# usnistgov/alignn

Measured on AMD Instinct MI355X. Metric: graphs/sec (train fwd+bwd), batch=64 JARVIS-DFT crystals, 4+4 ALIGNN layers, higher is better.
Workload: dtype f32 (projections: split-product MFMA - 3 fp16-slice or 6 bf16-slice products, fp32 accumulate, fp32-grade error)

## Files before the change

alignn_amd/csrc/gemm_dw.hip:

```cpp
#include <type_traits>
#include <utility>

#include "common.h"
#include "../../include/alignn_hip.h"

#ifndef DW_ABL
#define DW_ABL 0
#endif
#ifndef DW_TRACE
#define DW_TRACE 0
#endif
#ifndef DW_NS
#define DW_NS 4
#endif
#ifndef DW_IL
#define DW_IL 0
#endif
#ifndef DW_PP
#define DW_PP 0
#endif
#if DW_TRACE
__device__ unsigned long long dw_trace_buf[256 * 16];
#endif

#ifndef DW_GRID_DEFAULT
#define DW_GRID_DEFAULT 224
#endif

namespace {

typedef float f32x16 __attribute__((ext_vector_type(16)));
typedef _Float16 f16x8 __attribute__((ext_vector_type(8)));
typedef short s16x4 __attribute__((__vector_size__(4 * sizeof(short))));
typedef short s16x8 __attribute__((__vector_size__(8 * sizeof(short))));

constexpr int H = 256;
constexpr int R = 64;
constexpr int NW = 8, NTH = NW * 64;
constexpr int NS = DW_NS;
constexpr int SLOT = 16384;
constexpr int GBUF = 0;
constexpr int RING = GBUF + R * 1024;
constexpr int PATCH = RING + NS * SLOT;
constexpr int PLD = 68, PATCH_W = 8 * PLD * 4;
constexpr int NSTAT = PATCH + NW * PATCH_W;
constexpr int LDS_BYTES = NSTAT + 4 * H * 4;
static_assert(LDS_BYTES <= 160 * 1024, "one workgroup per CU");

template <int NE>
struct Sched {
    static constexpr int EST = NE == 2 ? 8 : 4, E0 = 12, STEPS = E0 + EST, NSL = 20 + (NE > 0 ? EST : 0), STORES = 8 / EST;
    static_assert(NSL % NS == 0, "ring positions are compile-time constants");
    int w0[STEPS], ws[STEPS];
    int g0, gs;
    int prologue;
    static constexpr int cons(int s) { return s < 4 ? 1 : s < E0 ? 2 : (NE > 0 ? 1 : 0); }
    static constexpr int first(int s) { return s <= 4 ? s : s <= E0 ? 4 + 2 * (s - 4) : 20 + (s - E0) * cons(E0); }
    static constexpr int fill_lo(int s) { return (s == 0 ? first(STEPS - 1) - NSL : first(s - 1)) + NS; }
    static constexpr int fill_n(int s) { return s == 0 ? cons(STEPS - 1) : cons(s - 1); }
    static constexpr int slot_ops(int n) {
        n = ((n % NSL) + NSL) % NSL;
        if ((DW_ABL & 32) && n < 4) return 0;
        if ((DW_ABL & 1) && n >= 4 && n < 20) return 0;
        if ((DW_ABL & 2) && n >= 20) return 0;
        return 2;
    }
    static constexpr int g_ops() { return (DW_ABL & 64) ? 0 : 8; }
    static constexpr int store_ops() { return (DW_ABL & 16) ? 0 : STORES; }
    static constexpr Sched make() {
        Sched r{};
        constexpr int TILES = 3;
        int end_op[(TILES + 1) * NSL + NS] = {};
        int g_end[TILES + 2] = {};
        int ops = 0;
        g_end[0] = (ops += g_ops());
        r.prologue = fill_lo(0);
        for (int n = 0; n < r.prologue; ++n) end_op[n] = (ops += slot_ops(n));
        int w[TILES][STEPS] = {};
        int gw[TILES] = {};
        for (int t = 0; t < TILES; ++t) {
            gw[t] = ops - g_end[t];
            for (int s = 0; s < STEPS; ++s) {
                if (cons(s) > 0) w[t][s] = ops - end_op[t * NSL + first(s) + cons(s) - 1];
                for (int k = 0; k < fill_n(s); ++k) end_op[t * NSL + fill_lo(s) + k] = (ops += slot_ops(fill_lo(s) + k));
                if (s == E0) g_end[t + 1] = (ops += g_ops());
                if (s >= E0) ops += store_ops();
            }
        }
        for (int s = 0; s < STEPS; ++s) r.w0[s] = w[0][s], r.ws[s] = w[2][s];
        r.g0 = gw[0], r.gs = gw[2];
        for (int s = 0; s < STEPS; ++s)
            if (w[1][s] != w[2][s]) r.gs = -1;
        if (gw[1] != gw[2]) r.gs = -1;
        return r;
    }
};

template <int NE>
inline constexpr Sched<NE> kSched = Sched<NE>::make();

template <int N>
__device__ __forceinline__ void wait_vmcnt() {
    static_assert(N >= 0 && N < 64, "vmcnt is a 6-bit counter");
    asm volatile("s_waitcnt vmcnt(%0)" ::"n"(N) : "memory");
}
__device__ __forceinline__ void block_barrier() {
    asm volatile("s_waitcnt lgkmcnt(0)" ::: "memory");
    __builtin_amdgcn_s_barrier();
    asm volatile("" ::: "memory");
}
__device__ __forceinline__ void dma16(const void* sbase, unsigned lane_off, unsigned char* lds_wave_base) {
    asm volatile("s_mov_b32 m0, %0\n\ts_nop 0\n\tglobal_load_lds_dwordx4 %1, %2"
                 :
                 : "s"((unsigned)(size_t)lds_wave_base), "v"(lane_off), "s"(sbase)
                 : "memory");
}
template <int B, int E, class F>
__device__ __forceinline__ void static_for(F&& f) {
    if constexpr (B < E) {
        f(std::integral_constant<int, B>{});
        static_for<B + 1, E>(f);
    }
}

__device__ __forceinline__ float f16_scale(float amax) {
    const int e = (int)((__float_as_uint(amax) >> 23) & 255u);
    if (e == 0 || e == 255) return 1.0f;
    int se = 268 - e;
    se = se > 254 ? 254 : se;
    return __uint_as_float((unsigned)se << 23);
}
__device__ __forceinline__ void slice8(const float4& a, const float4& b, float s, uint4& hp, uint4& lp) {
    const float x[8] = {a.x, a.y, a.z, a.w, b.x, b.y, b.z, b.w};
    float xs[8];
    f16x8 h;
#pragma unroll
    for (int j = 0; j < 8; ++j) {
        xs[j] = x[j] * s;
        h[j] = (_Float16)xs[j];
    }
    hp = __builtin_bit_cast(uint4, h);
    const unsigned hw[4] = {hp.x, hp.y, hp.z, hp.w};
    unsigned lw[4];
#pragma unroll
    for (int p = 0; p < 4; ++p) {
        asm("v_fma_mixlo_f16 %0, %1, 1.0, -%2 op_sel:[0,0,0] op_sel_hi:[0,0,1]" : "=v"(lw[p]) : "v"(xs[2 * p]), "v"(hw[p]));
        asm("v_fma_mixhi_f16 %0, %1, 1.0, -%2 op_sel:[0,0,1] op_sel_hi:[0,0,1]" : "+v"(lw[p]) : "v"(xs[2 * p + 1]), "v"(hw[p]));
    }
    lp = make_uint4(lw[0], lw[1], lw[2], lw[3]);
}

__host__ __device__ constexpr int swz(int row) { return ((row & 3) << 2) | ((row >> 2) & 3); }

template <int OFF>
__device__ __forceinline__ f16x8 tr_operand(const unsigned char* p0, const unsigned char* p1) {
    typedef __attribute__((address_space(3))) s16x4* lp;
    const s16x4 a = __builtin_amdgcn_ds_read_tr16_b64_v4i16((lp)(p0 + OFF));
    const s16x4 b = __builtin_amdgcn_ds_read_tr16_b64_v4i16((lp)(p1 + OFF));
    return __builtin_bit_cast(f16x8, __builtin_shufflevector(a, b, 0, 1, 2, 3, 4, 5, 6, 7));
}

struct DwArgs {
    const float* G;
    int64_t ldg;
    const float* Y;
    int64_t ldy;
    const unsigned char* Wt;
    const float *g_amax, *y_amax, *w_amax;
    const float* addend;
    int64_t ldadd;
    float* C;
    int64_t ldc;
    const float* xn;
    int64_t ldxn;
    const float* nstat;
    float* red_partial;
    float* dw_ws;
    int64_t M;
    int tiles;
};

template <bool HAS_ADD, bool BNRED>
__global__ __launch_bounds__(NTH) __attribute__((amdgpu_waves_per_eu(2, 2))) void gemm_dw_kernel(DwArgs g) {
    constexpr int NE = (HAS_ADD ? 1 : 0) + (BNRED ? 1 : 0);
    using S = Sched<NE>;
    static_assert(kSched<NE>.gs >= 0, "the operation sequence is periodic from the second tile on");
    extern __shared__ __attribute__((aligned(1024))) unsigned char smem[];
    const int t = threadIdx.x, lane = t & 63;
    const int wave = __builtin_amdgcn_readfirstlane(t >> 6);
    const int il = lane & 31, half = lane >> 5;
    const int wm = wave >> 2, wn = wave & 3;
    const int wf = wave >> 1, wc = wave & 1;
    const int grid = gridDim.x;
    const int J = (g.tiles - (int)blockIdx.x + grid - 1) / grid;

    const float sg = f16_scale(*g.g_amax), sy = f16_scale(*g.y_amax);
    const float inv_sg = 1.0f / sg, inv_sw = 1.0f / f16_scale(*g.w_amax);
    const float inv_dw = (1.0f / sg) * (1.0f / sy);

    if constexpr (BNRED) {
        for (int i = t; i < 4 * H / 4; i += NTH) *reinterpret_cast<float4*>(smem + NSTAT + i * 16) = f4_ld(g.nstat + i * 4);
    }

    const unsigned lane16 = lane * 16;
    struct TileRef {
        int64_t m0;
        int last;
    };
    auto tile_ref = [&](int tl) {
        tl = tl < g.tiles ? tl : g.tiles - 1;
        const int64_t m0 = (int64_t)tl * R;
        return TileRef{m0, (int)(g.M - 1 - m0 < R - 1 ? g.M - 1 - m0 : R - 1)};
    };
    auto row_dma = [&](const float* base, int64_t ld, const TileRef& tr, int row, unsigned char* dst) {
        row = row < tr.last ? row : tr.last;
        dma16(base + tr.m0 * ld, lane16 + (unsigned)(row * (int)ld) * 4u, dst);
    };
    auto lane_dma = [&](const float* base, int64_t ld, const TileRef& tr, int row, unsigned col_b, unsigned char* dst) {
        row = row < tr.last ? row : tr.last;
        dma16(base + tr.m0 * ld, col_b + (unsigned)(row * (int)ld) * 4u, dst);
    };
    auto issue_G = [&](const TileRef& tr) {
        if constexpr (S::g_ops() == 0) return;
#pragma unroll
        for (int i = 0; i < 8; ++i) row_dma(g.G, g.ldg, tr, wave * 8 + i, smem + GBUF + (wave * 8 + i) * 1024);
    };
    auto issue_slot = [&](auto nc, const TileRef& tr, int only = -1) {
        constexpr int n = decltype(nc)::value;
        if constexpr (S::slot_ops(n) == 0) return;
        unsigned char* dst = smem + RING + (n % NS) * SLOT;
#pragma unroll
        for (int i = 0; i < 2; ++i) {
            if (only >= 0 && only != i) continue;
            const int lr = 2 * wave + i;
            if constexpr (n < 4) {
                row_dma(g.Y, g.ldy, tr, 16 * n + lr, dst + lr * 1024);
            } else if constexpr (n < 20) {
                dma16(g.Wt + (n - 4) * SLOT, lane16 + (unsigned)lr * 1024u, dst + lr * 1024);
            } else {
                constexpr int e = n - 20;
                const int r4 = lane >> 4;
                const unsigned col_b = (unsigned)(64 * (wave & 3)) * 4u + (unsigned)(lane & 15) * 16u;
                if constexpr (NE == 1) {
                    const int trow = 32 * (wave >> 2) + 8 * e + 4 * i + r4;
                    if constexpr (HAS_ADD)
                        lane_dma(g.addend, g.ldadd, tr, trow, col_b, dst + wave * 2048 + i * 1024);
                    else
                        lane_dma(g.xn, g.ldxn, tr, trow, col_b, dst + wave * 2048 + i * 1024);
                } else {
                    const int trow = 32 * (wave >> 2) + 4 * e + r4;
                    if (i == 0)
                        lane_dma(g.addend, g.ldadd, tr, trow, col_b, dst + wave * 2048);
                    else
                        lane_dma(g.xn, g.ldxn, tr, trow, col_b, dst + wave * 2048 + 1024);
                }
            }
        }
    };

    auto opaque_lane = [&]() {
        int l = lane;
        asm volatile("" : "+v"(l));
        return l;
    };

    f32x16 acc_dw[2][4], acc_c[2];
#pragma unroll
    for (int a = 0; a < 2; ++a)
#pragma unroll
        for (int b = 0; b < 4; ++b)
#pragma unroll
            for (int r = 0; r < 16; ++r) acc_dw[a][b][r] = 0.0f;
    float4 s0 = f4_zero(), s1 = f4_zero();

    int tile = blockIdx.x;
    {
        const TileRef tr0 = tile_ref(tile);
        issue_G(tr0);
        static_for<0, kSched<NE>.prologue>([&](auto nc) { issue_slot(nc, tr0); });
    }

#if DW_TRACE
    unsigned long long tr_t[8] = {0, 0, 0, 0, 0, 0, 0, 0}, tr_w[3] = {0, 0, 0}, tr_b[3] = {0, 0, 0};
    int tr_j = 0;
#define DW_STAMP(i) do { if (tr_j == 2) tr_t[i] = __builtin_readcyclecounter(); } while (0)
#define DW_WAIT(ph, stmt) do { const unsigned long long t0_ = __builtin_readcyclecounter(); stmt; if (tr_j == 2) tr_w[ph] += __builtin_readcyclecounter() - t0_; } while (0)
#define DW_BARRIER(ph) do { const unsigned long long t0_ = __builtin_readcyclecounter(); block_barrier(); if (tr_j == 2) tr_b[ph] += __builtin_readcyclecounter() - t0_; } while (0)
#else
#define DW_STAMP(i) do { } while (0)
#define DW_WAIT(ph, stmt) stmt
#define DW_BARRIER(ph) block_barrier()
#endif
    f16x8 yah[2], yal[2], ybh[4], ybl[4];
    f16x8 wah[2], wal[2], wbh[2][2], wbl[2][2];
    int ta_off[2], tb_off[2], a_base, b_off[2];
    auto y_reads = [&](auto sc) {
        constexpr int s = decltype(sc)::value;
        int ta0 = ta_off[0], ta1 = ta_off[1], tb0 = tb_off[0], tb1 = tb_off[1];
        asm volatile("" : "+v"(ta0), "+v"(ta1), "+v"(tb0), "+v"(tb1));
#pragma unroll
        for (int a = 0; a < 2; ++a) {
            const unsigned char* p0 = smem + (ta0 ^ (a << 6));
            const unsigned char* p1 = smem + (ta1 ^ (a << 6));
            yah[a] = tr_operand<s * SLOT>(p0, p1);
            yal[a] = tr_operand<s * SLOT + 512>(p0, p1);
        }
#pragma unroll
        for (int b = 0; b < 4; ++b) {
            const unsigned char* p0 = smem + (tb0 ^ (b << 6));
            const unsigned char* p1 = smem + (tb1 ^ (b << 6));
            ybh[b] = tr_operand<(s % NS) * SLOT>(p0, p1);
            ybl[b] = tr_operand<(s % NS) * SLOT + 512>(p0, p1);
        }
    };
    auto no_il = [](auto) {};
    auto y_mfma = [&](auto&& between) {
        if constexpr (!(DW_ABL & 8)) {
#define DW_PASS(AA, BB)                                                                       \
    _Pragma("unroll") for (int a = 0; a < 2; ++a) _Pragma("unroll") for (int b = 0; b < 4; ++b) \
        acc_dw[a][b] = __builtin_amdgcn_mfma_f32_32x32x16_f16(AA[a], BB[b], acc_dw[a][b], 0, 0, 0);
            DW_PASS(yal, ybh)
            between(std::integral_constant<int, 0>{});
            DW_PASS(yah, ybl)
            between(std::integral_constant<int, 1>{});
            DW_PASS(yah, ybh)
#undef DW_PASS
        } else {
            acc_dw[0][0][0] += (float)yah[0][0] + (float)ybh[0][0] + (float)yal[1][0] + (float)ybl[3][0];
            between(std::integral_constant<int, 0>{});
            between(std::integral_constant<int, 1>{});
        }
    };
    auto w_reads = [&](auto ktc) {
        constexpr int kt0 = decltype(ktc)::value;
        int ab = a_base;
        asm volatile("" : "+v"(ab));
#pragma unroll
        for (int j = 0; j < 2; ++j) {
            const unsigned char* slot = smem + RING + ((kt0 + j + 4) % NS) * SLOT;
            const unsigned char* ap = smem + (ab ^ ((kt0 + j) << 5));
            wah[j] = __builtin_bit_cast(f16x8, *reinterpret_cast<const uint4*>(ap));
            wal[j] = __builtin_bit_cast(f16x8, *reinterpret_cast<const uint4*>(ap + 512));
#pragma unroll
            for (int b = 0; b < 2; ++b) {
                wbh[j][b] = __builtin_bit_cast(f16x8, *reinterpret_cast<const uint4*>(slot + b_off[b]));
                wbl[j][b] = __builtin_bit_cast(f16x8, *reinterpret_cast<const uint4*>(slot + b_off[b] + 8192));
            }
        }
    };
    auto w_mfma = [&](auto&& between) {
        static_for<0, 2>([&](auto jc) {
            constexpr int j = decltype(jc)::value;
            if constexpr (!(DW_ABL & 4)) {
                acc_c[0] = __builtin_amdgcn_mfma_f32_32x32x16_f16(wah[j], wbh[j][0], acc_c[0], 0, 0, 0);
                acc_c[1] = __builtin_amdgcn_mfma_f32_32x32x16_f16(wah[j], wbh[j][1], acc_c[1], 0, 0, 0);
                acc_c[0] = __builtin_amdgcn_mfma_f32_32x32x16_f16(wah[j], wbl[j][0], acc_c[0], 0, 0, 0);
                between(std::integral_constant<int, 2 * j>{});
                acc_c[1] = __builtin_amdgcn_mfma_f32_32x32x16_f16(wah[j], wbl[j][1], acc_c[1], 0, 0, 0);
                acc_c[0] = __builtin_amdgcn_mfma_f32_32x32x16_f16(wal[j], wbh[j][0], acc_c[0], 0, 0, 0);
                acc_c[1] = __builtin_amdgcn_mfma_f32_32x32x16_f16(wal[j], wbh[j][1], acc_c[1], 0, 0, 0);
                between(std::integral_constant<int, 2 * j + 1>{});
            } else {
                acc_c[0][0] += (float)wah[j][0] + (float)wal[j][0] + (float)wbh[j][0][0] + (float)wbl[j][1][0];
                between(std::integral_constant<int, 2 * j>{});
                between(std::integral_constant<int, 2 * j + 1>{});
            }
        });
    };

    auto tile_body = [&](auto first_c, auto lead_c) {
        constexpr bool FIRST = decltype(first_c)::value, lead = decltype(lead_c)::value;
        DW_STAMP(0);
        const TileRef cur = tile_ref(tile), nxt = tile_ref(tile + grid);
        const int64_t m0 = cur.m0;
        DW_WAIT(0, (wait_vmcnt<FIRST ? kSched<NE>.g0 : kSched<NE>.gs>()));
        DW_STAMP(1);
        {
            const int l = opaque_lane();
            const int wslot = l >> 1, wsub = (l & 1) * 8;
#pragma unroll
            for (int i0 = 0; i0 < 8; i0 += 4) {
                float4 v[4];
#pragma unroll
                for (int i = 0; i < 4; ++i) v[i] = *reinterpret_cast<const float4*>(smem + GBUF + (wave * 8 + i0 + i) * 1024 + l * 16);
#pragma unroll
                for (int i = 0; i < 4; i += 2) {
                    uint4 hp, lp;
                    slice8(v[i], v[i + 1], sg, hp, lp);
                    const int ra = wave * 8 + i0 + i, rb = ra + 1;
                    unsigned char* pa = smem + GBUF + ra * 1024 + ((wslot ^ swz(ra)) << 4) + wsub;
                    unsigned char* pb = smem + GBUF + rb * 1024 + ((wslot ^ swz(rb)) << 4) + wsub;
                    *reinterpret_cast<uint2*>(pa) = make_uint2(hp.x, hp.y);
                    *reinterpret_cast<uint2*>(pa + 512) = make_uint2(lp.x, lp.y);
                    *reinterpret_cast<uint2*>(pb) = make_uint2(hp.z, hp.w);
                    *reinterpret_cast<uint2*>(pb + 512) = make_uint2(lp.z, lp.w);
                }
            }
        }
        {
            const int l = opaque_lane(), grp = l >> 4, i16 = l & 15;
#pragma unroll
            for (int h = 0; h < 2; ++h) {
                const int row = 8 * (grp >> 1) + 4 * h + (i16 >> 2);
                const int sl = 2 * (grp & 1) + ((i16 >> 1) & 1);
                ta_off[h] = GBUF + row * 1024 + (((8 * wf + sl) ^ swz(row)) << 4) + (i16 & 1) * 8;
                tb_off[h] = RING + row * 1024 + (((16 * wc + sl) ^ swz(row)) << 4) + (i16 & 1) * 8;
            }
        }
        auto y_convert = [&](auto sc) {
            constexpr int s = decltype(sc)::value;
            DW_WAIT(0, (wait_vmcnt<FIRST ? kSched<NE>.w0[s] : kSched<NE>.ws[s]>()));
            unsigned char* slot = smem + RING + (s % NS) * SLOT;
            const int ra = 2 * wave, rb = ra + 1;
            const int l = opaque_lane();
            float4 va = *reinterpret_cast<const float4*>(slot + ra * 1024 + l * 16);
            float4 vb = *reinterpret_cast<const float4*>(slot + rb * 1024 + l * 16);
            const float ka = m0 + 16 * s + ra < g.M ? 1.0f : 0.0f, kb = m0 + 16 * s + rb < g.M ? 1.0f : 0.0f;
            va = f4_scale(va, ka);
            vb = f4_scale(vb, kb);
            uint4 hp, lp;
            slice8(va, vb, sy, hp, lp);
            unsigned char* pa = slot + ra * 1024 + ((((l >> 1) ^ swz(ra))) << 4) + (l & 1) * 8;
            unsigned char* pb = slot + rb * 1024 + ((((l >> 1) ^ swz(rb))) << 4) + (l & 1) * 8;
            *reinterpret_cast<uint2*>(pa) = make_uint2(hp.x, hp.y);
            *reinterpret_cast<uint2*>(pa + 512) = make_uint2(lp.x, lp.y);
            *reinterpret_cast<uint2*>(pb) = make_uint2(hp.z, hp.w);
            *reinterpret_cast<uint2*>(pb + 512) = make_uint2(lp.z, lp.w);
        };
        auto fills = [&](auto sc) {
            constexpr int s = decltype(sc)::value;
            static_for<0, S::fill_n(s)>([&](auto kc) {
                constexpr int n = S::fill_lo(s) + decltype(kc)::value;
                issue_slot(std::integral_constant<int, n % S::NSL>{}, n >= S::NSL ? nxt : cur);
            });
        };
        auto fill_piece = [&](auto sc, auto kc) {
            constexpr int s = decltype(sc)::value, k = decltype(kc)::value;
            if constexpr (k < 2 * S::fill_n(s)) {
                constexpr int n = S::fill_lo(s) + k / 2;
                __builtin_amdgcn_sched_barrier(0);
                issue_slot(std::integral_constant<int, n % S::NSL>{}, n >= S::NSL ? nxt : cur, k % 2);
                __builtin_amdgcn_sched_barrier(0);
            }
        };
        DW_STAMP(2);
        y_convert(std::integral_constant<int, 0>{});
        static_for<0, 4>([&](auto sc) {
            constexpr int s = decltype(sc)::value;
            DW_BARRIER(0);
#if DW_PP
            if constexpr (lead) {
                fills(sc);
                y_reads(sc);
                if constexpr (s < 3) y_convert(std::integral_constant<int, s + 1>{});
            } else {
                if constexpr (s > 0) y_mfma(no_il);
            }
            block_barrier();
            if constexpr (lead) {
                y_mfma(no_il);
            } else {
                fills(sc);
                y_reads(sc);
                if constexpr (s < 3) y_convert(std::integral_constant<int, s + 1>{});
            }
#elif DW_IL
            y_reads(sc);
            y_mfma([&](auto kc) { fill_piece(sc, kc); });
            if constexpr (s < 3) y_convert(std::integral_constant<int, s + 1>{});
#else
            fills(sc);
            y_reads(sc);
            y_mfma(no_il);
            if constexpr (s < 3) y_convert(std::integral_constant<int, s + 1>{});
#endif
        });
#pragma unroll
        for (int b = 0; b < 2; ++b)
#pragma unroll
            for (int r = 0; r < 16; ++r) acc_c[b][r] = 0.0f;
        {
            const int l = opaque_lane(), il = l & 31, half = l >> 5;
            const int a_row = 32 * wm + il;
            a_base = GBUF + a_row * 1024 + ((half ^ swz(a_row)) << 4);
#pragma unroll
            for (int b = 0; b < 2; ++b) {
                const int n = 64 * wn + 32 * b + il;
                b_off[b] = n * 32 + ((half ^ ((n >> 3) & 1)) << 4);
            }
        }
        static_for<4, S::E0>([&](auto sc) {
            constexpr int s = decltype(sc)::value, kt0 = 2 * (s - 4);
            if (s == 4) DW_STAMP(3);
            DW_WAIT(1, (wait_vmcnt<FIRST ? kSched<NE>.w0[s] : kSched<NE>.ws[s]>()));
            DW_BARRIER(1);
#if DW_PP
            if constexpr (lead) {
                fills(sc);
                w_reads(std::integral_constant<int, kt0>{});
            } else {
                if constexpr (kt0 == 0)
                    y_mfma(no_il);
                else
                    w_mfma(no_il);
            }
            block_barrier();
            if constexpr (lead) {
                w_mfma(no_il);
            } else {
                fills(sc);
                w_reads(std::integral_constant<int, kt0>{});
            }
#elif DW_IL
            w_reads(std::integral_constant<int, kt0>{});
            w_mfma([&](auto kc) { fill_piece(sc, kc); });
#else
            fills(sc);
            w_reads(std::integral_constant<int, kt0>{});
            w_mfma(no_il);
#endif
        });
        const int last_row = cur.last;
        float* c_t = g.C + m0 * g.ldc;
        const int le = opaque_lane();
        const int prow_e = le >> 4, pc4 = (le & 15) * 4, ecol = 64 * wn + pc4, il = le & 31, half = le >> 5;
        float* patch = reinterpret_cast<float*>(smem + PATCH + wave * PATCH_W);
        static_for<S::E0, S::STEPS>([&](auto sc) {
            constexpr int s = decltype(sc)::value, e = s - S::E0;
            constexpr int QR = 32 / S::EST;
            constexpr int q = QR == 8 ? e : e / 2, hf = e & 1;
            constexpr int n_slot = 20 + e;
            if (e == 0) DW_STAMP(4);
            if constexpr (NE > 0) DW_WAIT(2, (wait_vmcnt<FIRST ? kSched<NE>.w0[s] : kSched<NE>.ws[s]>()));
            if constexpr (e == 0) DW_BARRIER(2);
            if constexpr (e == 0 && DW_PP && !lead) w_mfma(no_il);
            fills(sc);
            if constexpr (e == 0) issue_G(nxt);
            const unsigned char* mine = smem + RING + (n_slot % NS) * SLOT + wave * 2048;
#pragma unroll
            for (int nb = 0; nb < 2; ++nb)
#pragma unroll
                for (int k = 0; k < 4; ++k)
                    patch[(k + 4 * (QR == 8 ? half : (half ^ hf))) * PLD + 32 * nb + il] = acc_c[nb][4 * q + k];
#pragma unroll
            for (int i = 0; i < QR / 4; ++i) {
                const int pr = prow_e + 4 * i;
                const int rrel = 32 * wm + QR * e + pr;
                const int rowc = rrel < last_row ? rrel : last_row;
                float4 v = f4_ld(patch + pr * PLD + pc4);
                v = f4_scale(f4_scale(v, inv_sg), inv_sw);
                const int e_off = (NE == 2 ? prow_e : pr) * 256 + pc4 * 4;
                if constexpr (HAS_ADD) v = f4_add(v, *reinterpret_cast<const float4*>(mine + e_off));
                if constexpr (BNRED) {
                    const float4 xv = *reinterpret_cast<const float4*>(mine + e_off + (NE == 2 ? 1024 : 0));
                    const float4 xc = f4_sub(xv, *reinterpret_cast<const float4*>(smem + NSTAT + ecol * 4));
                    const float4 z = f4_fma(xc, *reinterpret_cast<const float4*>(smem + NSTAT + 2 * H * 4 + ecol * 4),
                                            *reinterpret_cast<const float4*>(smem + NSTAT + 3 * H * 4 + ecol * 4));
                    float4 gz = make_float4(v.x * dsilu_f(z.x), v.y * dsilu_f(z.y), v.z * dsilu_f(z.z), v.w * dsilu_f(z.w));
                    gz = rrel <= last_row ? gz : f4_zero();
                    s0 = f4_add(s0, gz);
                    s1 = f4_fma(gz, xc, s1);
                }
                if (!(DW_ABL & 16) || v.x == 12345.678f) f4_sts<true>(c_t + (rowc * (int)g.ldc + ecol), v);
                if constexpr (BNRED) __builtin_amdgcn_sched_barrier(0);
            }
        });
        DW_STAMP(5);
#if DW_TRACE
        ++tr_j;
#endif
    };
    auto run_tiles = [&](auto lead_c) {
        tile_body(std::true_type{}, lead_c);
        tile += grid;
        for (int j = 1; j < J; ++j, tile += grid) tile_body(std::false_type{}, lead_c);
    };
    if (!DW_PP || wave < 4)
        run_tiles(std::true_type{});
    else
        run_tiles(std::false_type{});
#if DW_TRACE
    if (threadIdx.x == 0 && blockIdx.x < 256) {
        unsigned long long* o = dw_trace_buf + blockIdx.x * 16;
        for (int i = 0; i < 6; ++i) o[i] = tr_t[i];
        for (int i = 0; i < 3; ++i) o[6 + i] = tr_w[i], o[9 + i] = tr_b[i];
    }
#endif

    wait_vmcnt<0>();
    {
        float* out = g.dw_ws + (size_t)blockIdx.x * (H * H);
#pragma unroll
        for (int a = 0; a < 2; ++a)
#pragma unroll
            for (int b = 0; b < 4; ++b)
#pragma unroll
                for (int r = 0; r < 16; ++r) {
                    const int f = 64 * wf + 32 * a + (r & 3) + 8 * (r >> 2) + 4 * half, c = 128 * wc + 32 * b + il;
                    out[f * H + c] = acc_dw[a][b][r] * inv_dw;
                }
    }
    if constexpr (BNRED) {
        const int ecol = 64 * wn + (lane & 15) * 4;
        float4 a0 = s0, a1 = s1;
#pragma unroll
        for (int d = 16; d < 64; d <<= 1) {
            a0 = f4_add(a0, make_float4(__shfl_xor(a0.x, d), __shfl_xor(a0.y, d), __shfl_xor(a0.z, d), __shfl_xor(a0.w, d)));
            a1 = f4_add(a1, make_float4(__shfl_xor(a1.x, d), __shfl_xor(a1.y, d), __shfl_xor(a1.z, d), __shfl_xor(a1.w, d)));
        }
        if (lane < 16) {
            a1 = f4_mul(a1, f4_ld(g.nstat + H + ecol));
            const size_t slab = (size_t)blockIdx.x * 2 + wm;
            f4_st(g.red_partial + (slab * 2 + 0) * H + ecol, a0);
            f4_st(g.red_partial + (slab * 2 + 1) * H + ecol, a1);
        }
    }
}

__global__ __launch_bounds__(1024) void dw_slab_reduce_kernel(const float* __restrict__ ws, int splits, float* __restrict__ out,
                                                              int64_t ldo) {
    __shared__ double sh[16][64][4];
    const int64_t count = H * H;
    const int64_t idx = ((int64_t)blockIdx.x * 64 + threadIdx.x) * 4;
    double s[4] = {0.0, 0.0, 0.0, 0.0};
    for (int k = threadIdx.y; k < splits; k += 16) {
        const float4 v = f4_ld(ws + (int64_t)k * count + idx);
        s[0] += (double)v.x, s[1] += (double)v.y, s[2] += (double)v.z, s[3] += (double)v.w;
    }
    double* mine = sh[threadIdx.y][threadIdx.x];
    mine[0] = s[0], mine[1] = s[1], mine[2] = s[2], mine[3] = s[3];
    __syncthreads();
    if (threadIdx.y == 0) {
        double t0 = 0.0, t1 = 0.0, t2 = 0.0, t3 = 0.0;
#pragma unroll 4
        for (int k = 0; k < 16; ++k) {
            const double* p = sh[k][threadIdx.x];
            t0 += p[0], t1 += p[1], t2 += p[2], t3 += p[3];
        }
        f4_st(out + (idx / H) * ldo + (idx % H), make_float4((float)t0, (float)t1, (float)t2, (float)t3));
    }
}

constexpr int kGridMax = 256;
inline int dw_grid_cap() {
    static const int cap = [] {
        const char* e = getenv("ALIGNN_AMD_DW_GRID");
        int v = e ? atoi(e) : DW_GRID_DEFAULT;
        v = v < 8 ? 8 : (v > kGridMax ? kGridMax : v);
        return v & ~7;
    }();
    return cap;
}
inline int dw_grid(int64_t M) {
    const int64_t tiles = (M + R - 1) / R;
    const int cap = dw_grid_cap();
    return (int)(tiles < cap ? tiles : cap);
}
inline bool a16(const void* p) { return (reinterpret_cast<uintptr_t>(p) & 15) == 0; }

}

#if DW_TRACE
extern "C" int alignn_dw_trace_read(void* host, size_t bytes) {
    return (int)hipMemcpyFromSymbol(host, HIP_SYMBOL(dw_trace_buf), bytes < sizeof(dw_trace_buf) ? bytes : sizeof(dw_trace_buf));
}
#endif

extern "C" {

int alignn_gemm_dgrad_wgrad_supported(int64_t M, int N, int K) {
    return (N == H && K == H && M >= 4096 && (M + R - 1) / R < ((int64_t)1 << 30)) ? 1 : 0;
}
int alignn_gemm_dgrad_wgrad_slabs(int64_t M) { return dw_grid(M); }
size_t alignn_gemm_dgrad_wgrad_workspace(int64_t M) { return (size_t)dw_grid(M) * H * H * sizeof(float); }

int alignn_gemm_dgrad_wgrad_f16x3(const float* G, int64_t ldg, const float* g_amax, const float* Y, int64_t ldy, const float* y_amax,
                                  const void* Wt_split, const float* w_amax, const float* addend, int64_t ldadd, float* C,
                                  int64_t ldc, const float* Xn, int64_t ldxn, const float* nstat, float* red_partial, float* dW,
                                  int64_t lddw, int64_t M, void* workspace, size_t workspace_bytes, alignn_stream_t stream) {
    if (!alignn_gemm_dgrad_wgrad_supported(M, H, H) || G == nullptr || Y == nullptr || Wt_split == nullptr || C == nullptr ||
        dW == nullptr || g_amax == nullptr || y_amax == nullptr || w_amax == nullptr)
        return (int)hipErrorInvalidValue;
    if ((ldg & 3) || (ldy & 3) || (ldc & 3) || (lddw & 3) || !a16(G) || !a16(Y) || !a16(C) || !a16(dW) || !a16(Wt_split) ||
        (addend && ((ldadd & 3) || !a16(addend))))
        return (int)hipErrorInvalidValue;
    const bool bnred = Xn != nullptr;
    if (bnred && (nstat == nullptr || red_partial == nullptr || (ldxn & 3) || !a16(Xn) || !a16(nstat) || !a16(red_partial)))
        return (int)hipErrorInvalidValue;
    if (workspace == nullptr || !a16(workspace) || workspace_bytes < alignn_gemm_dgrad_wgrad_workspace(M))
        return (int)hipErrorInvalidValue;
    const int grid = dw_grid(M);
    DwArgs g{G, ldg, Y, ldy, (const unsigned char*)Wt_split, g_amax, y_amax, w_amax, addend, ldadd, C, ldc, Xn, ldxn, nstat,
             red_partial, (float*)workspace, M, (int)((M + R - 1) / R)};
    static bool attr_set = false;
    if (!attr_set) {
        const void* fns[] = {(const void*)gemm_dw_kernel<false, false>, (const void*)gemm_dw_kernel<true, false>,
                             (const void*)gemm_dw_kernel<false, true>, (const void*)gemm_dw_kernel<true, true>};
        for (const void* fn : fns) {
            hipError_t e = hipFuncSetAttribute(fn, hipFuncAttributeMaxDynamicSharedMemorySize, LDS_BYTES);
            if (e != hipSuccess) return (int)e;
        }
        attr_set = true;
    }
    hipStream_t st = (hipStream_t)stream;
    if (addend != nullptr && bnred)
        hipLaunchKernelGGL((gemm_dw_kernel<true, true>), dim3(grid), dim3(NTH), LDS_BYTES, st, g);
    else if (addend != nullptr)
        hipLaunchKernelGGL((gemm_dw_kernel<true, false>), dim3(grid), dim3(NTH), LDS_BYTES, st, g);
    else if (bnred)
        hipLaunchKernelGGL((gemm_dw_kernel<false, true>), dim3(grid), dim3(NTH), LDS_BYTES, st, g);
    else
        hipLaunchKernelGGL((gemm_dw_kernel<false, false>), dim3(grid), dim3(NTH), LDS_BYTES, st, g);
    ALIGNN_CHECK_LAUNCH();
    hipLaunchKernelGGL(dw_slab_reduce_kernel, dim3(H * H / 256), dim3(64, 16), 0, st, (const float*)workspace, grid, dW, lddw);
    ALIGNN_CHECK_LAUNCH();
    return 0;
}

}
```

Measured before the change: 4455.

## Overlap dW GEMM epilogue of previous tile with next tile's Y-phase MFMAs

Adds an overlapped-epilogue schedule (DW_OVL, on by default for the addend-only variant). The previous tile's output scaling, addend add and stores are deferred and interleaved into the Y-phase MFMA loop of the following tile. Addend rows are streamed through the ring alongside the Y slots, and the remaining epilogue is drained after the tile loop. The goal is to hide the serial epilogue step per tile. In exchange the compile-time vmcnt schedule gets more complex, and the final tile pays an un-overlapped drain.

```diff
diff --git a/alignn_amd/csrc/gemm_dw.hip b/alignn_amd/csrc/gemm_dw.hip
--- a/alignn_amd/csrc/gemm_dw.hip
+++ b/alignn_amd/csrc/gemm_dw.hip
@@ -18,6 +18,9 @@
 #endif
 #ifndef DW_PP
 #define DW_PP 0
+#endif
+#ifndef DW_OVL
+#define DW_OVL 1
 #endif
 #if DW_TRACE
 __device__ unsigned long long dw_trace_buf[256 * 16];
@@ -47,22 +50,26 @@
 constexpr int LDS_BYTES = NSTAT + 4 * H * 4;
 static_assert(LDS_BYTES <= 160 * 1024, "one workgroup per CU");
 
-template <int NE>
+template <int NE, bool OVL = false>
 struct Sched {
-    static constexpr int EST = NE == 2 ? 8 : 4, E0 = 12, STEPS = E0 + EST, NSL = 20 + (NE > 0 ? EST : 0), STORES = 8 / EST;
+    static constexpr int EST = OVL ? 0 : (NE == 2 ? 8 : 4), E0 = 12, STEPS = E0 + EST, YS = OVL ? 1 + NE : 1, W0 = 4 * YS;
+    static constexpr int NSL = W0 + 16 + (!OVL && NE > 0 ? EST : 0), STORES = OVL ? 2 : 8 / EST;
     static_assert(NSL % NS == 0, "ring positions are compile-time constants");
     int w0[STEPS], ws[STEPS];
+    int we0[4], wes[4];
     int g0, gs;
     int prologue;
-    static constexpr int cons(int s) { return s < 4 ? 1 : s < E0 ? 2 : (NE > 0 ? 1 : 0); }
-    static constexpr int first(int s) { return s <= 4 ? s : s <= E0 ? 4 + 2 * (s - 4) : 20 + (s - E0) * cons(E0); }
+    static constexpr int cons(int s) { return s < 4 ? YS : s < E0 ? 2 : (NE > 0 ? 1 : 0); }
+    static constexpr int waited(int s) { return OVL && s < 4 ? 1 : cons(s); }
+    static constexpr int first(int s) { return s <= 4 ? YS * s : s <= E0 ? W0 + 2 * (s - 4) : W0 + 16 + (s - E0) * cons(E0); }
     static constexpr int fill_lo(int s) { return (s == 0 ? first(STEPS - 1) - NSL : first(s - 1)) + NS; }
     static constexpr int fill_n(int s) { return s == 0 ? cons(STEPS - 1) : cons(s - 1); }
+    static constexpr int kind(int n) { return n < W0 ? (n % YS == 0 ? 0 : 2) : n < W0 + 16 ? 1 : 2; }
     static constexpr int slot_ops(int n) {
         n = ((n % NSL) + NSL) % NSL;
-        if ((DW_ABL & 32) && n < 4) return 0;
-        if ((DW_ABL & 1) && n >= 4 && n < 20) return 0;
-        if ((DW_ABL & 2) && n >= 20) return 0;
+        if ((DW_ABL & 32) && kind(n) == 0) return 0;
+        if ((DW_ABL & 1) && kind(n) == 1) return 0;
+        if ((DW_ABL & 2) && kind(n) == 2) return 0;
         return 2;
     }
     static constexpr int g_ops() { return (DW_ABL & 64) ? 0 : 8; }
@@ -76,28 +83,36 @@
         g_end[0] = (ops += g_ops());
         r.prologue = fill_lo(0);
         for (int n = 0; n < r.prologue; ++n) end_op[n] = (ops += slot_ops(n));
-        int w[TILES][STEPS] = {};
+        int w[TILES][STEPS] = {}, we[TILES][4] = {};
         int gw[TILES] = {};
         for (int t = 0; t < TILES; ++t) {
             gw[t] = ops - g_end[t];
             for (int s = 0; s < STEPS; ++s) {
-                if (cons(s) > 0) w[t][s] = ops - end_op[t * NSL + first(s) + cons(s) - 1];
+                if (cons(s) > 0) w[t][s] = ops - end_op[t * NSL + first(s) + waited(s) - 1];
                 for (int k = 0; k < fill_n(s); ++k) end_op[t * NSL + fill_lo(s) + k] = (ops += slot_ops(fill_lo(s) + k));
-                if (s == E0) g_end[t + 1] = (ops += g_ops());
-                if (s >= E0) ops += store_ops();
-            }
+                if (!OVL && s == E0) g_end[t + 1] = (ops += g_ops());
+                if (!OVL && s >= E0) ops += store_ops();
+                if (OVL && s < 4) {
+                    if (NE > 0) we[t][s] = ops - end_op[t * NSL + first(s) + NE];
+                    if (t > 0) ops += store_ops();
+                }
+            }
+            if (OVL) g_end[t + 1] = (ops += g_ops());
         }
         for (int s = 0; s < STEPS; ++s) r.w0[s] = w[0][s], r.ws[s] = w[2][s];
+        for (int s = 0; s < 4; ++s) r.we0[s] = we[0][s], r.wes[s] = we[2][s];
         r.g0 = gw[0], r.gs = gw[2];
         for (int s = 0; s < STEPS; ++s)
             if (w[1][s] != w[2][s]) r.gs = -1;
+        for (int s = 0; s < 4; ++s)
+            if (we[1][s] != we[2][s]) r.gs = -1;
         if (gw[1] != gw[2]) r.gs = -1;
         return r;
     }
 };
 
-template <int NE>
-inline constexpr Sched<NE> kSched = Sched<NE>::make();
+template <int NE, bool OVL = false>
+inline constexpr Sched<NE, OVL> kSched = Sched<NE, OVL>::make();
 
 template <int N>
 __device__ __forceinline__ void wait_vmcnt() {
@@ -180,11 +195,14 @@
     int tiles;
 };
 
+static_assert(!(DW_OVL && (DW_PP || DW_IL)), "the overlapped epilogue is a form of the lock-step schedule");
+
 template <bool HAS_ADD, bool BNRED>
 __global__ __launch_bounds__(NTH) __attribute__((amdgpu_waves_per_eu(2, 2))) void gemm_dw_kernel(DwArgs g) {
     constexpr int NE = (HAS_ADD ? 1 : 0) + (BNRED ? 1 : 0);
-    using S = Sched<NE>;
-    static_assert(kSched<NE>.gs >= 0, "the operation sequence is periodic from the second tile on");
+    constexpr bool OVL = (DW_OVL == 1 && HAS_ADD && !BNRED) || (DW_OVL == 2 && NE == 1);
+    using S = Sched<NE, OVL>;
+    static_assert(kSched<NE, OVL>.gs >= 0, "the operation sequence is periodic from the second tile on");
     extern __shared__ __attribute__((aligned(1024))) unsigned char smem[];
     const int t = threadIdx.x, lane = t & 63;
     const int wave = __builtin_amdgcn_readfirstlane(t >> 6);
@@ -225,7 +243,7 @@
 #pragma unroll
         for (int i = 0; i < 8; ++i) row_dma(g.G, g.ldg, tr, wave * 8 + i, smem + GBUF + (wave * 8 + i) * 1024);
     };
-    auto issue_slot = [&](auto nc, const TileRef& tr, int only = -1) {
+    auto issue_slot = [&](auto nc, const TileRef& tr, const TileRef& tre, int only = -1) {
         constexpr int n = decltype(nc)::value;
         if constexpr (S::slot_ops(n) == 0) return;
         unsigned char* dst = smem + RING + (n % NS) * SLOT;
@@ -233,10 +251,18 @@
         for (int i = 0; i < 2; ++i) {
             if (only >= 0 && only != i) continue;
             const int lr = 2 * wave + i;
-            if constexpr (n < 4) {
-                row_dma(g.Y, g.ldy, tr, 16 * n + lr, dst + lr * 1024);
-            } else if constexpr (n < 20) {
-                dma16(g.Wt + (n - 4) * SLOT, lane16 + (unsigned)lr * 1024u, dst + lr * 1024);
+            if constexpr (S::kind(n) == 0) {
+                row_dma(g.Y, g.ldy, tr, 16 * (n / S::YS) + lr, dst + lr * 1024);
+            } else if constexpr (S::kind(n) == 1) {
+                dma16(g.Wt + (n - S::W0) * SLOT, lane16 + (unsigned)lr * 1024u, dst + lr * 1024);
+            } else if constexpr (OVL) {
+                const int r4 = lane >> 4;
+                const unsigned col_b = (unsigned)(64 * (wave & 3)) * 4u + (unsigned)(lane & 15) * 16u;
+                const int trow = 32 * (wave >> 2) + 8 * (n / S::YS) + 4 * i + r4;
+                if constexpr (HAS_ADD && n % S::YS == 1)
+                    lane_dma(g.addend, g.ldadd, tre, trow, col_b, dst + wave * 2048 + i * 1024);
+                else
+                    lane_dma(g.xn, g.ldxn, tre, trow, col_b, dst + wave * 2048 + i * 1024);
             } else {
                 constexpr int e = n - 20;
                 const int r4 = lane >> 4;
@@ -277,7 +303,7 @@
     {
         const TileRef tr0 = tile_ref(tile);
         issue_G(tr0);
-        static_for<0, kSched<NE>.prologue>([&](auto nc) { issue_slot(nc, tr0); });
+        static_for<0, kSched<NE, OVL>.prologue>([&](auto nc) { issue_slot(nc, tr0, tr0); });
     }
 
 #if DW_TRACE
@@ -309,8 +335,8 @@
         for (int b = 0; b < 4; ++b) {
             const unsigned char* p0 = smem + (tb0 ^ (b << 6));
             const unsigned char* p1 = smem + (tb1 ^ (b << 6));
-            ybh[b] = tr_operand<(s % NS) * SLOT>(p0, p1);
-            ybl[b] = tr_operand<(s % NS) * SLOT + 512>(p0, p1);
+            ybh[b] = tr_operand<(S::YS * s % NS) * SLOT>(p0, p1);
+            ybl[b] = tr_operand<(S::YS * s % NS) * SLOT + 512>(p0, p1);
         }
     };
     auto no_il = [](auto) {};
@@ -337,7 +363,7 @@
         asm volatile("" : "+v"(ab));
 #pragma unroll
         for (int j = 0; j < 2; ++j) {
-            const unsigned char* slot = smem + RING + ((kt0 + j + 4) % NS) * SLOT;
+            const unsigned char* slot = smem + RING + ((kt0 + j + S::W0) % NS) * SLOT;
             const unsigned char* ap = smem + (ab ^ ((kt0 + j) << 5));
             wah[j] = __builtin_bit_cast(f16x8, *reinterpret_cast<const uint4*>(ap));
             wal[j] = __builtin_bit_cast(f16x8, *reinterpret_cast<const uint4*>(ap + 512));
@@ -368,12 +394,46 @@
         });
     };
 
+    auto ovl_epi = [&](auto qc, auto partc, const TileRef& pt) {
+        constexpr int q = decltype(qc)::value, part = decltype(partc)::value;
+        const int le = opaque_lane();
+        const int prow_e = le >> 4, pc4 = (le & 15) * 4, ecol = 64 * wn + pc4, il = le & 31, half = le >> 5;
+        float* patch = reinterpret_cast<float*>(smem + PATCH + wave * PATCH_W);
+        if constexpr (part == 0) {
+#pragma unroll
+            for (int nb = 0; nb < 2; ++nb)
+#pragma unroll
+                for (int k = 0; k < 4; ++k) patch[(k + 4 * half) * PLD + 32 * nb + il] = acc_c[nb][4 * q + k];
+        }
+        const int pr = prow_e + 4 * part;
+        const int rrel = 32 * wm + 8 * q + pr;
+        const int rowc = rrel < pt.last ? rrel : pt.last;
+        float4 v = f4_ld(patch + pr * PLD + pc4);
+        v = f4_scale(f4_scale(v, inv_sg), inv_sw);
+        const int e_off = pr * 256 + pc4 * 4;
+        const unsigned char* mine_a = smem + RING + ((S::YS * q + 1) % NS) * SLOT + wave * 2048;
+        const unsigned char* mine_x = smem + RING + ((S::YS * q + NE) % NS) * SLOT + wave * 2048;
+        if constexpr (HAS_ADD) v = f4_add(v, *reinterpret_cast<const float4*>(mine_a + e_off));
+        if constexpr (BNRED) {
+            const float4 xv = *reinterpret_cast<const float4*>(mine_x + e_off);
+            const float4 xc = f4_sub(xv, *reinterpret_cast<const float4*>(smem + NSTAT + ecol * 4));
+            const float4 z = f4_fma(xc, *reinterpret_cast<const float4*>(smem + NSTAT + 2 * H * 4 + ecol * 4),
+                                    *reinterpret_cast<const float4*>(smem + NSTAT + 3 * H * 4 + ecol * 4));
+            float4 gz = make_float4(v.x * dsilu_f(z.x), v.y * dsilu_f(z.y), v.z * dsilu_f(z.z), v.w * dsilu_f(z.w));
+            gz = rrel <= pt.last ? gz : f4_zero();
+            s0 = f4_add(s0, gz);
+            s1 = f4_fma(gz, xc, s1);
+        }
+        if (!(DW_ABL & 16) || v.x == 12345.678f) f4_sts<true>(g.C + pt.m0 * g.ldc + (rowc * (int)g.ldc + ecol), v);
+    };
+
     auto tile_body = [&](auto first_c, auto lead_c) {
         constexpr bool FIRST = decltype(first_c)::value, lead = decltype(lead_c)::value;
         DW_STAMP(0);
         const TileRef cur = tile_ref(tile), nxt = tile_ref(tile + grid);
+        const TileRef prv = tile_ref(FIRST ? tile : tile - grid);
         const int64_t m0 = cur.m0;
-        DW_WAIT(0, (wait_vmcnt<FIRST ? kSched<NE>.g0 : kSched<NE>.gs>()));
+        DW_WAIT(0, (wait_vmcnt<FIRST ? kSched<NE, OVL>.g0 : kSched<NE, OVL>.gs>()));
         DW_STAMP(1);
         {
             const int l = opaque_lane();
@@ -409,8 +469,8 @@
         }
         auto y_convert = [&](auto sc) {
             constexpr int s = decltype(sc)::value;
-            DW_WAIT(0, (wait_vmcnt<FIRST ? kSched<NE>.w0[s] : kSched<NE>.ws[s]>()));
-            unsigned char* slot = smem + RING + (s % NS) * SLOT;
+            DW_WAIT(0, (wait_vmcnt<FIRST ? kSched<NE, OVL>.w0[s] : kSched<NE, OVL>.ws[s]>()));
+            unsigned char* slot = smem + RING + (S::YS * s % NS) * SLOT;
             const int ra = 2 * wave, rb = ra + 1;
             const int l = opaque_lane();
             float4 va = *reinterpret_cast<const float4*>(slot + ra * 1024 + l * 16);
@@ -431,7 +491,7 @@
             constexpr int s = decltype(sc)::value;
             static_for<0, S::fill_n(s)>([&](auto kc) {
                 constexpr int n = S::fill_lo(s) + decltype(kc)::value;
-                issue_slot(std::integral_constant<int, n % S::NSL>{}, n >= S::NSL ? nxt : cur);
+                issue_slot(std::integral_constant<int, n % S::NSL>{}, n >= S::NSL ? nxt : cur, n >= S::NSL ? cur : prv);
             });
         };
         auto fill_piece = [&](auto sc, auto kc) {
@@ -439,7 +499,7 @@
             if constexpr (k < 2 * S::fill_n(s)) {
                 constexpr int n = S::fill_lo(s) + k / 2;
                 __builtin_amdgcn_sched_barrier(0);
-                issue_slot(std::integral_constant<int, n % S::NSL>{}, n >= S::NSL ? nxt : cur, k % 2);
+                issue_slot(std::integral_constant<int, n % S::NSL>{}, n >= S::NSL ? nxt : cur, n >= S::NSL ? cur : prv, k % 2);
                 __builtin_amdgcn_sched_barrier(0);
             }
         };
@@ -471,7 +531,17 @@
 #else
             fills(sc);
             y_reads(sc);
-            y_mfma(no_il);
+            if constexpr (OVL && !FIRST) {
+                y_mfma([&](auto kc) {
+                    constexpr int k = decltype(kc)::value;
+                    __builtin_amdgcn_sched_barrier(0);
+                    if constexpr (k == 0 && NE > 0) DW_WAIT(2, (wait_vmcnt<kSched<NE, OVL>.wes[s]>()));
+                    ovl_epi(sc, kc, prv);
+                    __builtin_amdgcn_sched_barrier(0);
+                });
+            } else {
+                y_mfma(no_il);
+            }
             if constexpr (s < 3) y_convert(std::integral_constant<int, s + 1>{});
 #endif
         });
@@ -492,7 +562,7 @@
         static_for<4, S::E0>([&](auto sc) {
             constexpr int s = decltype(sc)::value, kt0 = 2 * (s - 4);
             if (s == 4) DW_STAMP(3);
-            DW_WAIT(1, (wait_vmcnt<FIRST ? kSched<NE>.w0[s] : kSched<NE>.ws[s]>()));
+            DW_WAIT(1, (wait_vmcnt<FIRST ? kSched<NE, OVL>.w0[s] : kSched<NE, OVL>.ws[s]>()));
             DW_BARRIER(1);
 #if DW_PP
             if constexpr (lead) {
@@ -520,6 +590,12 @@
             w_mfma(no_il);
 #endif
         });
+        if constexpr (OVL) {
+            DW_STAMP(4);
+            DW_BARRIER(2);
+            issue_G(nxt);
+        }
+        if constexpr (!OVL) {
         const int last_row = cur.last;
         float* c_t = g.C + m0 * g.ldc;
         const int le = opaque_lane();
@@ -531,7 +607,7 @@
             constexpr int q = QR == 8 ? e : e / 2, hf = e & 1;
             constexpr int n_slot = 20 + e;
             if (e == 0) DW_STAMP(4);
-            if constexpr (NE > 0) DW_WAIT(2, (wait_vmcnt<FIRST ? kSched<NE>.w0[s] : kSched<NE>.ws[s]>()));
+            if constexpr (NE > 0) DW_WAIT(2, (wait_vmcnt<FIRST ? kSched<NE, OVL>.w0[s] : kSched<NE, OVL>.ws[s]>()));
             if constexpr (e == 0) DW_BARRIER(2);
             if constexpr (e == 0 && DW_PP && !lead) w_mfma(no_il);
             fills(sc);
@@ -565,6 +641,7 @@
                 if constexpr (BNRED) __builtin_amdgcn_sched_barrier(0);
             }
         });
+        }
         DW_STAMP(5);
 #if DW_TRACE
         ++tr_j;
@@ -579,6 +656,19 @@
         run_tiles(std::true_type{});
     else
         run_tiles(std::false_type{});
+    if constexpr (OVL) {
+        const TileRef last = tile_ref(tile - grid);
+        static_for<0, 4>([&](auto qc) {
+            constexpr int q = decltype(qc)::value;
+            static_for<1, 1 + NE>([&](auto ic) {
+                constexpr int n = S::YS * q + decltype(ic)::value;
+                if constexpr (n >= S::fill_lo(0)) issue_slot(std::integral_constant<int, n>{}, last, last);
+            });
+            wait_vmcnt<0>();
+            ovl_epi(qc, std::integral_constant<int, 0>{}, last);
+            ovl_epi(qc, std::integral_constant<int, 1>{}, last);
+        });
+    }
 #if DW_TRACE
     if (threadIdx.x == 0 && blockIdx.x < 256) {
         unsigned long long* o = dw_trace_buf + blockIdx.x * 16;
```

After: 4472, median of 6. Within noise of the previous version (+0.4%).
